# denix56/SI-Mamba

Hardware: AMD Instinct MI355X
Metric: point-clouds/sec (fwd+bwd) (higher is better)
Workload: dtype f32; 1 GPU; PointMamba classifier train step (FPS+kNN grouping, encoder, spectral SAST ordering, 12 Mamba blocks d=384 at L=1024, head, AdamW), 1024 pts -> 128 patches; global_batch=64, per_gpu_batch=64, npoints=1024, patches=128, mamba_seq_len=1024, parallelism=dp1, communicator_ranks=1, library_gemm=tuned solution table (si_mamba_amd/tuned/gemm_gfx950.csv)

## Files before the change

include/simamba.h:

```cpp
#ifndef SIMAMBA_H_
#define SIMAMBA_H_

#include <stddef.h>

#ifdef __cplusplus
extern "C" {
#endif

#define SIMAMBA_ABI_VERSION 9

#define SIMAMBA_F32  0
#define SIMAMBA_BF16 1

#define SIMAMBA_OK            0
#define SIMAMBA_E_NULLPTR    -1
#define SIMAMBA_E_SHAPE      -2
#define SIMAMBA_E_DTYPE      -3
#define SIMAMBA_E_DSTATE     -4
#define SIMAMBA_E_WIDTH      -5
#define SIMAMBA_E_WORKSPACE  -6
#define SIMAMBA_E_GROUPS     -7
#define SIMAMBA_E_ALIGN      -8
#define SIMAMBA_E_VARIANT    -9
#define SIMAMBA_E_BIAS       -10
// ... 74 lines not shown
                         void* stream);
int simamba_conv_xdt_proj_fwd(const void* x, const float* cw, const float* cb, const void* wx, const void* wdt,
                              void* xconv, void* xdbl, void* delta, int batch, int D, int seqlen, int S, int R,
                              int io_dtype, long long x_bstride, void* stream);

int simamba_seq_gather_fwd(const void* in, const int* idx, void* out, int batch, int channels, int G, int L,
                           long long out_bstride, int io_dtype, void* stream);
int simamba_seq_gather_bwd(const void* dout, const int* inv, void* din, int batch, int channels, int G, int L,
                           int R, long long dout_bstride, int io_dtype, void* stream);

int simamba_causal_conv1d_fwd(const void* x, const float* w, const float* bias, void* out,
                              int batch, int dim, int seqlen, int width, int silu,
                              int io_dtype, long long x_bstride, void* stream);
int simamba_causal_conv1d_bwd(const void* x, const float* w, const float* bias,
                              const void* dout, void* dx, float* dw, float* dbias,
                              int batch, int dim, int seqlen, int width, int silu,
                              int io_dtype, long long x_bstride, long long dx_bstride, void* stream);
long long simamba_causal_conv1d_bwd_workspace_floats(int batch, int dim, int seqlen, int width, int flags);
int simamba_causal_conv1d_bwd_ex(const void* x, const float* w, const float* bias,
                                 const void* dout, void* dx, float* dw, float* dbias,
                                 int batch, int dim, int seqlen, int width, int silu,
                                 int io_dtype, long long x_bstride, long long dx_bstride, int flags,
                                 float* workspace, long long workspace_floats, void* stream);

int simamba_add_layer_norm_grid(int batch, int rows_per_batch);
int simamba_add_layer_norm_fwd(const void* hidden, const float* residual, const float* rowscale,
                               const float* weight, const float* bias, float* residual_out,
                               void* normed, float* mean, float* rstd, int batch, int rows_per_batch,
                               int dim, float eps, int hidden_dtype, int out_dtype, void* stream);
int simamba_add_layer_norm_bwd(const void* dnormed, const float* dresidual_out,
                               const float* residual_out, const float* mean, const float* rstd,
                               const float* weight, const float* rowscale, float* dresidual,
                               void* dhidden, float* dwb_partial, int batch, int rows_per_batch,
                               int dim, int hidden_dtype, int out_dtype, void* stream);

#define SIMAMBA_NORM_RMS 1
int simamba_add_layer_norm_fwd_ex(const void* hidden, const float* residual, const float* rowscale,
                                  const float* weight, const float* bias, float* residual_out,
                                  void* normed, float* mean, float* rstd, int batch, int rows_per_batch,
                                  int dim, float eps, int hidden_dtype, int out_dtype, int flags, void* stream);
int simamba_add_layer_norm_bwd_ex(const void* dnormed, const float* dresidual_out,
                                  const float* residual_out, const float* mean, const float* rstd,
                                  const float* weight, const float* rowscale, float* dresidual,
                                  void* dhidden, float* dwb_partial, int batch, int rows_per_batch,
                                  int dim, int hidden_dtype, int out_dtype, int flags, void* stream);

// ... 203 lines not shown
```

si_mamba_amd/_lib.py:

```python
from __future__ import annotations

import ctypes
import os
from ctypes import c_char_p, c_float, c_int, c_longlong, c_size_t, c_uint, c_void_p

_HERE = os.path.dirname(os.path.abspath(__file__))
LIB_PATH = os.path.join(_HERE, "libsimamba_hip.so")

F32, BF16 = 0, 1

SPEC_SYMMETRIC = 0x01
SPEC_SELF_LOOP = 0x02
SPEC_BINARY = 0x04
SPEC_MATRIX_SYM = 0x08
SPEC_SMALLEST = 0x10
SPEC_SIGMA_MEAN = 0x20
SPEC_LARGE_G = 0x40
SPEC_MAX_G = 128
SPEC_MAX_G_LARGE = 512

SCAN_AUTO, SCAN_ROWSCAN, SCAN_LPC2, SCAN_LPC4, SCAN_MIX = 0, 1, 2, 4, 6
CKPT_ROW, CKPT_SEQ = 128, 16
BWD_DETERMINISTIC = 1
NORM_RMS = 1
# ... 34 lines not shown
                                              _LL, _LL, _LL, _LL, _LL, c_int, c_int, _P, _LL, _P]),
    "simamba_selective_scan_dt_fwd": (c_int, [_P, _P, _P, _P, _P, _P, _P, _P, _P, _P,
                                              c_int, c_int, c_int, c_int, c_int, c_int,
                                              _LL, _LL, _LL, c_int, c_int, _P]),
    "simamba_selective_scan_dt_bwd": (c_int, [_P, _P, _P, _P, _P, _P, _P, _P, _P,
                                              _P, _P, _P, _P, _P, _P, _P, _P,
                                              c_int, c_int, c_int, c_int, c_int, c_int,
                                              _LL, _LL, _LL, _LL, _P]),
    "simamba_selective_scan_dt_bwd_ex": (c_int, [_P, _P, _P, _P, _P, _P, _P, _P, _P,
                                                 _P, _P, _P, _P, _P, _P, _P, _P,
                                                 c_int, c_int, c_int, c_int, c_int, c_int,
                                                 _LL, _LL, _LL, _LL, c_int, _P, _LL, _P]),
    "simamba_xdt_proj_fwd": (c_int, [_P, _P, _P, _P, _P, c_int, c_int, c_int, c_int, c_int, c_int, _LL, _P]),
    "simamba_conv_xdt_proj_fwd": (c_int, [_P, _P, _P, _P, _P, _P, _P, _P, c_int, c_int, c_int, c_int, c_int, c_int, _LL,
                                          _P]),
    "simamba_seq_gather_fwd": (c_int, [_P, _P, _P, c_int, c_int, c_int, c_int, _LL, c_int, _P]),
    "simamba_seq_gather_bwd": (c_int, [_P, _P, _P, c_int, c_int, c_int, c_int, c_int, _LL, c_int, _P]),
    "simamba_causal_conv1d_fwd": (c_int, [_P, _P, _P, _P, c_int, c_int, c_int, c_int, c_int, c_int, _LL, _P]),
    "simamba_causal_conv1d_bwd": (c_int, [_P, _P, _P, _P, _P, _P, _P,
                                          c_int, c_int, c_int, c_int, c_int, c_int, _LL, _LL, _P]),
    "simamba_causal_conv1d_bwd_workspace_floats": (_LL, [c_int, c_int, c_int, c_int, c_int]),
    "simamba_causal_conv1d_bwd_ex": (c_int, [_P, _P, _P, _P, _P, _P, _P,
                                             c_int, c_int, c_int, c_int, c_int, c_int, _LL, _LL, c_int, _P, _LL, _P]),
    "simamba_add_layer_norm_grid": (c_int, [c_int, c_int]),
    "simamba_add_layer_norm_fwd": (c_int, [_P, _P, _P, _P, _P, _P, _P, _P, _P, c_int, c_int, c_int, c_float,
                                           c_int, c_int, _P]),
    "simamba_add_layer_norm_bwd": (c_int, [_P, _P, _P, _P, _P, _P, _P, _P, _P, _P, c_int, c_int, c_int,
                                           c_int, c_int, _P]),
    "simamba_add_layer_norm_fwd_ex": (c_int, [_P, _P, _P, _P, _P, _P, _P, _P, _P, c_int, c_int, c_int, c_float,
                                              c_int, c_int, c_int, _P]),
    "simamba_add_layer_norm_bwd_ex": (c_int, [_P, _P, _P, _P, _P, _P, _P, _P, _P, _P, c_int, c_int, c_int,
                                              c_int, c_int, c_int, _P]),
    "simamba_add_layer_norm_check_slots": (c_int, [_P, c_int, c_int]),
    "simamba_add_layer_norm_fwd_slots": (c_int, [_P, _P, _P, _P, _P, _P, _P, _P, _P, _P, c_int, _P, c_int, c_int, c_int,
                                                 c_int, c_float, c_int, c_int, c_int, _P]),
    "simamba_add_layer_norm_bwd_slots": (c_int, [_P, _P, _P, _P, _P, _P, _P, _P, _P, _P, _P, c_int, _P, c_int, c_int,
                                                 c_int, c_int, c_int, c_int, c_int, _P]),
    "simamba_out_proj_add_ln_fwd": (c_int, [_P, _P, _P, _P, _P, _P, _P, _P, _P, _P, c_int, c_int, c_int, c_int, c_float,
                                            c_int, _P]),
    "simamba_out_proj_add_ln_fwd_ex": (c_int, [_P, _P, _P, _P, _P, _P, _P, _P, _P, _P, c_int, c_int, c_int, c_int,
                                               c_float, c_int, c_int, _P]),
    "simamba_in_proj_fwd": (c_int, [_P, _P, _P, c_int, c_int, c_int, c_int, c_int, _P]),
    "simamba_bn_relu_grid": (c_int, [_LL]),
    "simamba_bn_relu_fwd": (c_int, [_P, _P, c_int, _P, _P, _P, _P, c_float, c_float, c_int, _P, _P, _P, _P, _LL, c_int,
                                    _LL, c_int, _P]),
    "simamba_bn_relu_bwd": (c_int, [_P, _P, _P, c_int, _P, _P, _P, _P, _P, _P, c_int, _P, _P, _P, _LL, c_int, _LL,
# ... 313 lines not shown
    step = scan_plan_step(batch, dim, seqlen, dstate, dtype, **operands)
    count("scan_ckpt_seq" if step == CKPT_SEQ else "scan_ckpt_row")
    if not need_grad:
        return step, None
    n = load().simamba_scan_ckpt_floats(batch, dim, seqlen, dstate, step)
    return step, (torch.empty(n, device=device, dtype=torch.float32) if n else None)


def scan_bwd_accumulators(batch, dim, seqlen, dstate, has_D, has_bias, device):
    import torch
    sizes = [dim * dstate, batch * dstate * seqlen, batch * dstate * seqlen, dim if has_D else 0,
             dim if has_bias else 0]
    flat = torch.empty(sum(sizes), device=device, dtype=torch.float32)
    parts, o = [], 0
    for n in sizes:
        parts.append(flat[o:o + n])
        o += n
    dA = parts[0].view(dim, dstate)
    dB = parts[1].view(batch, dstate, seqlen)
    dC = parts[2].view(batch, dstate, seqlen)
    return dA, dB, dC, (parts[3] if has_D else None), (parts[4] if has_bias else None)


_deterministic = [None]


def set_deterministic(on):
    _deterministic[0] = _tristate(on)


class deterministic(_Override):
    cell, coerce = _deterministic, staticmethod(_tristate)


def deterministic_enabled():
    if _deterministic[0] is not None:
        return _deterministic[0]
    import torch
    return torch.are_deterministic_algorithms_enabled()


def det_args(workspace_query, *dims, device):
    if not deterministic_enabled():
        return 0, None, 0
    import torch
    n_floats = workspace_query(*dims, BWD_DETERMINISTIC)
# ... 4 lines not shown
```

si_mamba_amd/csrc/add_norm.hip:

```cpp
#include "common.h"

namespace simamba {

constexpr int kLnThreads = 256;
constexpr int kLnMaxChunks = 8;

struct LnArgs {
  const void* hidden;
  const float* residual;
  const float* rowscale;
  const float* weight;
  const float* bias;
  float* residual_out;
  void* normed;
  float* mean;
  float* rstd;
  const void* dnormed;
  const float* dresidual_out;
  float* dresidual;
  void* dhidden;
  float* dwb_partial;
  const int* hidden_slot;
  const int* normed_slot;
  int hidden_batch, normed_batch;
  int batch, rows_per_batch, dim;
  float eps;
};

template <typename T>
__device__ __forceinline__ float4 ld4(const T* p) {
  const Pack<T, 4> pk = *reinterpret_cast<const Pack<T, 4>*>(p);
  return make_float4(to_f32<T>(pk.v[0]), to_f32<T>(pk.v[1]), to_f32<T>(pk.v[2]), to_f32<T>(pk.v[3]));
}
template <typename T>
__device__ __forceinline__ void st4(T* p, float4 v) {
  Pack<T, 4> pk;
  pk.v[0] = from_f32<T>(v.x); pk.v[1] = from_f32<T>(v.y); pk.v[2] = from_f32<T>(v.z); pk.v[3] = from_f32<T>(v.w);
  *reinterpret_cast<Pack<T, 4>*>(p) = pk;
}

__device__ __forceinline__ int ln_slot(const int* __restrict__ map, int b, int count) {
  if (!map) return b;
  const int s = __builtin_amdgcn_readfirstlane(map[b]);
  return (s >= 0 && s < count) ? s : -1;
}

struct LnRow {
  int b, hs, os;
};
__device__ __forceinline__ LnRow ln_row(const LnArgs& p, int row) {
  LnRow r;
  r.b = __builtin_amdgcn_readfirstlane(row / p.rows_per_batch);
  r.hs = ln_slot(p.hidden_slot, r.b, p.hidden_batch);
  r.os = ln_slot(p.normed_slot, r.b, p.normed_batch);
  return r;
}

template <typename TH, typename TO, int kChunks, bool kRms>
__global__ __launch_bounds__(kLnThreads) void add_ln_fwd_kernel(LnArgs p) {
  const bool slots = p.hidden_slot || p.normed_slot;
  const int lane = threadIdx.x & 63;
  const int wave_global = (blockIdx.x * kLnThreads + threadIdx.x) >> 6;
  const int nwaves = (gridDim.x * kLnThreads) >> 6;
  const int rows = p.batch * p.rows_per_batch;
  const int nch = p.dim >> 2;
  const TH* __restrict__ hg = static_cast<const TH*>(p.hidden);
  TO* __restrict__ og = static_cast<TO*>(p.normed);
  float4 w[kChunks], bs[kChunks];
#pragma unroll
  for (int k = 0; k < kChunks; ++k) {
    const int c = lane + 64 * k;
    w[k] = c < nch ? *reinterpret_cast<const float4*>(p.weight + 4 * c) : make_float4(0, 0, 0, 0);
    bs[k] = (!kRms && c < nch && p.bias) ? *reinterpret_cast<const float4*>(p.bias + 4 * c) : make_float4(0, 0, 0, 0);
  }
  const float inv_dim = 1.f / p.dim;
  LnRow next = (slots && wave_global < rows) ? ln_row(p, wave_global) : LnRow{0, 0, 0};
  for (int row = wave_global; row < rows; row += nwaves) {
    const size_t base = static_cast<size_t>(row) * p.dim;
    const float scale = (p.rowscale && p.residual) ? p.rowscale[row / p.rows_per_batch] : 1.f;
    size_t hbase = base, obase = base;
    bool has_h = true, has_o = true;
    if (slots) {
      const LnRow cur = next;
      const int ahead = row + nwaves;
      next = ln_row(p, ahead < rows ? ahead : row);
      const int r = __builtin_amdgcn_readfirstlane(row) - cur.b * p.rows_per_batch;
      has_h = cur.hs >= 0; has_o = cur.os >= 0;
      hbase = (static_cast<size_t>(has_h ? cur.hs : 0) * p.rows_per_batch + r) * p.dim;
      obase = (static_cast<size_t>(has_o ? cur.os : 0) * p.rows_per_batch + r) * p.dim;
    }
    float4 x[kChunks];
    float sum = 0.f;
#pragma unroll
    for (int k = 0; k < kChunks; ++k) {
      const int c = lane + 64 * k;
      if (c < nch) {
        float4 h;
        if (!has_h) {
          h = *reinterpret_cast<const float4*>(p.residual + base + 4 * c);
        } else {
          h = ld4<TH>(hg + hbase + 4 * c);
          if (p.residual) {
            const float4 r = *reinterpret_cast<const float4*>(p.residual + base + 4 * c);
            h.x = fmaf(h.x, scale, r.x); h.y = fmaf(h.y, scale, r.y);
            h.z = fmaf(h.z, scale, r.z); h.w = fmaf(h.w, scale, r.w);
          }
        }
        if (p.residual_out) *reinterpret_cast<float4*>(p.residual_out + base + 4 * c) = h;
        x[k] = h;
        sum += (h.x + h.y) + (h.z + h.w);
      } else {
        x[k] = make_float4(0, 0, 0, 0);
// ... 30 lines not shown
}

template <typename TH, typename TO, int kChunks, bool kRms>
__global__ __launch_bounds__(kLnThreads) void add_ln_bwd_kernel(LnArgs p) {
  const bool slots = p.hidden_slot || p.normed_slot;
  extern __shared__ float sred[];
  const int lane = threadIdx.x & 63;
  const int wave = threadIdx.x >> 6;
  const int wave_global = (blockIdx.x * kLnThreads + threadIdx.x) >> 6;
  const int nwaves = (gridDim.x * kLnThreads) >> 6;
  const int rows = p.batch * p.rows_per_batch;
  const int nch = p.dim >> 2;
  const TO* __restrict__ dyg = static_cast<const TO*>(p.dnormed);
  TH* __restrict__ dhg = static_cast<TH*>(p.dhidden);
  float4 w[kChunks], dw[kChunks], db[kChunks];
#pragma unroll
  for (int k = 0; k < kChunks; ++k) {
    const int c = lane + 64 * k;
    w[k] = c < nch ? *reinterpret_cast<const float4*>(p.weight + 4 * c) : make_float4(0, 0, 0, 0);
    dw[k] = make_float4(0, 0, 0, 0);
    db[k] = make_float4(0, 0, 0, 0);
  }
  const float inv_dim = 1.f / p.dim;
  LnRow next = (slots && wave_global < rows) ? ln_row(p, wave_global) : LnRow{0, 0, 0};
  for (int row = wave_global; row < rows; row += nwaves) {
    const size_t base = static_cast<size_t>(row) * p.dim;
    size_t hbase = base, obase = base;
    bool has_h = true, has_o = true;
    if (slots) {
      const LnRow cur = next;
      const int ahead = row + nwaves;
      next = ln_row(p, ahead < rows ? ahead : row);
      const int r = __builtin_amdgcn_readfirstlane(row) - cur.b * p.rows_per_batch;
      has_h = cur.hs >= 0; has_o = cur.os >= 0;
      hbase = (static_cast<size_t>(has_h ? cur.hs : 0) * p.rows_per_batch + r) * p.dim;
      obase = (static_cast<size_t>(has_o ? cur.os : 0) * p.rows_per_batch + r) * p.dim;
    }
    if (!has_o) {
      const float scale = (p.rowscale && dhg) ? p.rowscale[row / p.rows_per_batch] : 1.f;
#pragma unroll
      for (int k = 0; k < kChunks; ++k) {
        const int c = lane + 64 * k;
        if (c < nch) {
          const float4 dx = p.dresidual_out ? *reinterpret_cast<const float4*>(p.dresidual_out + base + 4 * c)
                                            : make_float4(0, 0, 0, 0);
          if (p.dresidual) *reinterpret_cast<float4*>(p.dresidual + base + 4 * c) = dx;
          if (dhg && has_h)
            st4<TH>(dhg + hbase + 4 * c, make_float4(dx.x * scale, dx.y * scale, dx.z * scale, dx.w * scale));
        }
      }
      continue;
    }
    const float mean = kRms ? 0.f : p.mean[row], rstd = p.rstd[row];
    float4 xh[kChunks], g[kChunks];
    float s1 = 0.f, s2 = 0.f;
#pragma unroll
    for (int k = 0; k < kChunks; ++k) {
      const int c = lane + 64 * k;
      if (c < nch) {
        const float4 x = *reinterpret_cast<const float4*>(p.residual_out + base + 4 * c);
        const float4 dy = ld4<TO>(dyg + obase + 4 * c);
        xh[k] = make_float4((x.x - mean) * rstd, (x.y - mean) * rstd, (x.z - mean) * rstd, (x.w - mean) * rstd);
        g[k] = make_float4(dy.x * w[k].x, dy.y * w[k].y, dy.z * w[k].z, dy.w * w[k].w);
        dw[k].x = fmaf(dy.x, xh[k].x, dw[k].x); dw[k].y = fmaf(dy.y, xh[k].y, dw[k].y);
        dw[k].z = fmaf(dy.z, xh[k].z, dw[k].z); dw[k].w = fmaf(dy.w, xh[k].w, dw[k].w);
        db[k].x += dy.x; db[k].y += dy.y; db[k].z += dy.z; db[k].w += dy.w;
        s1 += (g[k].x + g[k].y) + (g[k].z + g[k].w);
        s2 += (g[k].x * xh[k].x + g[k].y * xh[k].y) + (g[k].z * xh[k].z + g[k].w * xh[k].w);
      } else {
        xh[k] = make_float4(0, 0, 0, 0);
        g[k] = make_float4(0, 0, 0, 0);
      }
    }
    const float c1 = kRms ? 0.f : wave_allreduce_sum(s1) * inv_dim;
    const float c2 = wave_allreduce_sum(s2) * inv_dim;
    const float scale = (p.rowscale && dhg) ? p.rowscale[row / p.rows_per_batch] : 1.f;
#pragma unroll
    for (int k = 0; k < kChunks; ++k) {
      const int c = lane + 64 * k;
      if (c < nch) {
        float4 dx;
        dx.x = (g[k].x - c1 - xh[k].x * c2) * rstd;
        dx.y = (g[k].y - c1 - xh[k].y * c2) * rstd;
        dx.z = (g[k].z - c1 - xh[k].z * c2) * rstd;
        dx.w = (g[k].w - c1 - xh[k].w * c2) * rstd;
        if (p.dresidual_out) {
          const float4 r = *reinterpret_cast<const float4*>(p.dresidual_out + base + 4 * c);
          dx.x += r.x; dx.y += r.y; dx.z += r.z; dx.w += r.w;
        }
        if (p.dresidual) *reinterpret_cast<float4*>(p.dresidual + base + 4 * c) = dx;
        if (dhg && has_h)
          st4<TH>(dhg + hbase + 4 * c, make_float4(dx.x * scale, dx.y * scale, dx.z * scale, dx.w * scale));
      }
    }
  }
  float* mine = sred + wave * 2 * p.dim;
#pragma unroll
  for (int k = 0; k < kChunks; ++k) {
    const int c = lane + 64 * k;
    if (c < nch) {
      *reinterpret_cast<float4*>(mine + 4 * c) = dw[k];
      if (!kRms) *reinterpret_cast<float4*>(mine + p.dim + 4 * c) = db[k];
    }
  }
  __syncthreads();
  float* out = p.dwb_partial + static_cast<size_t>(blockIdx.x) * 2 * p.dim;
  for (int i = threadIdx.x; i < (kRms ? 1 : 2) * p.dim; i += kLnThreads) {
    float v = 0.f;
#pragma unroll
    for (int wv = 0; wv < kLnThreads / 64; ++wv) v += sred[wv * 2 * p.dim + i];
    out[i] = v;
  }
}

static int ln_grid(int rows) {
  int g = (rows + 3) / 4;
  return g < 1 ? 1 : (g > 1024 ? 1024 : g);
}

template <typename TH, typename TO, bool kRms>
static int launch_ln(const LnArgs& a, bool bwd, int grid, hipStream_t s) {
  const int chunks = ((a.dim >> 2) + 63) / 64;
#define SIMAMBA_LN_CASE(K)                                                                                      \
  if (chunks <= K) {                                                                                             \
    if (bwd)                                                                                                     \
      hipLaunchKernelGGL((add_ln_bwd_kernel<TH, TO, K, kRms>), dim3(grid), dim3(kLnThreads),                     \
                         sizeof(float) * (kLnThreads / 64) * 2 * a.dim, s, a);                                   \
    else                                                                                                         \
      hipLaunchKernelGGL((add_ln_fwd_kernel<TH, TO, K, kRms>), dim3(grid), dim3(kLnThreads), 0, s, a);           \
    return static_cast<int>(hipGetLastError());                                                                  \
  }
  SIMAMBA_LN_CASE(1)
  SIMAMBA_LN_CASE(2)
  SIMAMBA_LN_CASE(4)
  SIMAMBA_LN_CASE(8)
#undef SIMAMBA_LN_CASE
  return SIMAMBA_E_SHAPE;
}

template <typename TH, typename TO>
static int launch_ln(const LnArgs& a, bool bwd, bool rms, int grid, hipStream_t s) {
  return rms ? launch_ln<TH, TO, true>(a, bwd, grid, s) : launch_ln<TH, TO, false>(a, bwd, grid, s);
}

static int dispatch_ln(const LnArgs& a, bool bwd, bool rms, int grid, int hidden_dtype, int out_dtype, hipStream_t s) {
  if (hidden_dtype == SIMAMBA_F32 && out_dtype == SIMAMBA_F32) return launch_ln<float, float>(a, bwd, rms, grid, s);
  if (hidden_dtype == SIMAMBA_BF16 && out_dtype == SIMAMBA_BF16)
    return launch_ln<bf16_t, bf16_t>(a, bwd, rms, grid, s);
  if (hidden_dtype == SIMAMBA_F32 && out_dtype == SIMAMBA_BF16) return launch_ln<float, bf16_t>(a, bwd, rms, grid, s);
  if (hidden_dtype == SIMAMBA_BF16 && out_dtype == SIMAMBA_F32) return launch_ln<bf16_t, float>(a, bwd, rms, grid, s);
  return SIMAMBA_E_DTYPE;
}
// ... 126 lines not shown
```

si_mamba_amd/csrc/det_reduce.h:

```cpp
#pragma once
#include <hip/hip_runtime.h>

namespace simamba {

struct DetSumJob {
  const float* part;
  float* out;
  long long kstride;
  long long n;
  int K;
};

constexpr int kDetSumMaxJobs = 5;

int det_sum_launch(const DetSumJob* jobs, int njobs, hipStream_t s);

}
```

si_mamba_amd/csrc/det_reduce.hip:

```cpp
#include "det_reduce.h"

namespace simamba {

constexpr int kDetSumThreads = 256;
constexpr int kDetSumPerBlock = 4 * kDetSumThreads;

struct DetSumArgs {
  DetSumJob job[kDetSumMaxJobs];
  int vec[kDetSumMaxJobs];
  int blk0[kDetSumMaxJobs + 1];
  int njobs;
};

__global__ __launch_bounds__(kDetSumThreads) void det_sum_kernel(DetSumArgs a) {
  const int blk = blockIdx.x;
  int j = 0;
#pragma unroll
  for (int q = 1; q < kDetSumMaxJobs; ++q) j = (q < a.njobs && blk >= a.blk0[q]) ? q : j;
  const float* __restrict__ part = a.job[j].part;
  float* __restrict__ out = a.job[j].out;
  const long long ks = a.job[j].kstride, n = a.job[j].n;
  const int K = a.job[j].K;
  const long long i0 = (static_cast<long long>(blk - a.blk0[j]) * kDetSumThreads + threadIdx.x) * 4;
  if (i0 >= n) return;
  if (a.vec[j] && i0 + 4 <= n) {
    const float* p = part + i0;
    float4 acc = make_float4(0.f, 0.f, 0.f, 0.f);
    int k = 0;
    for (; k + 4 <= K; k += 4) {
      float4 v[4];
#pragma unroll
      for (int m = 0; m < 4; ++m) v[m] = *reinterpret_cast<const float4*>(p + (k + m) * ks);
#pragma unroll
      for (int m = 0; m < 4; ++m) {
        acc.x += v[m].x; acc.y += v[m].y; acc.z += v[m].z; acc.w += v[m].w;
      }
    }
    for (; k < K; ++k) {
      const float4 v = *reinterpret_cast<const float4*>(p + k * ks);
      acc.x += v.x; acc.y += v.y; acc.z += v.z; acc.w += v.w;
    }
    *reinterpret_cast<float4*>(out + i0) = acc;
    return;
  }
  for (long long i = i0; i < n && i < i0 + 4; ++i) {
    float acc = 0.f;
    for (int k = 0; k < K; ++k) acc += part[k * ks + i];
    out[i] = acc;
  }
}

int det_sum_launch(const DetSumJob* jobs, int njobs, hipStream_t s) {
  DetSumArgs a{};
  int blocks = 0, m = 0;
  for (int i = 0; i < njobs && m < kDetSumMaxJobs; ++i) {
    if (jobs[i].n <= 0) continue;
    a.job[m] = jobs[i];
    a.vec[m] = (reinterpret_cast<uintptr_t>(jobs[i].part) & 15u) == 0 && (reinterpret_cast<uintptr_t>(jobs[i].out) & 15u) == 0 &&
               jobs[i].kstride % 4 == 0;
    a.blk0[m] = blocks;
    blocks += static_cast<int>((jobs[i].n + kDetSumPerBlock - 1) / kDetSumPerBlock);
    ++m;
  }
  if (!m) return static_cast<int>(hipSuccess);
  a.njobs = m;
  for (int q = m; q <= kDetSumMaxJobs; ++q) a.blk0[q] = blocks;
  hipLaunchKernelGGL(det_sum_kernel, dim3(blocks), dim3(kDetSumThreads), 0, s, a);
  return static_cast<int>(hipGetLastError());
}

}
```

si_mamba_amd/mamba_inner.py:

```python
from __future__ import annotations

import torch

from . import _lib


def _w(t, dtype):
    return t if t.dtype == dtype else t.to(dtype)


def _wx(W, X):
    return torch.bmm(W.unsqueeze(0).expand(X.shape[0], -1, -1), X)


def _xw(X, W):
    return torch.bmm(X, W.unsqueeze(0).expand(X.shape[0], -1, -1))


def _sum_bmm(X, Y):
    return torch.bmm(X, Y).sum(0, dtype=torch.float32)


class InProjFn(torch.autograd.Function):

    @staticmethod
    def forward(ctx, hidden, weight, bias):
        io = hidden.dtype
        if torch.is_autocast_enabled("cuda"):
            io = torch.get_autocast_dtype("cuda")
            hidden = hidden.to(io)
        wc = _w(weight, io)
        xz = tokens_times_weight(hidden, wc) if bias is None else _wx(wc, hidden.transpose(1, 2))
        if bias is not None:
            xz = xz + _w(bias, io)[None, :, None]
        ctx.save_for_backward(hidden, weight)
        ctx.wc = wc
        ctx.has_bias = bias is not None
        return xz

    @staticmethod
    def backward(ctx, dxz):
        hidden, weight = ctx.saved_tensors
        io = hidden.dtype
        dxz = dxz.to(io)
        dh = _xw(dxz.transpose(1, 2), ctx.wc) if ctx.needs_input_grad[0] else None
        dw = _sum_bmm(dxz, hidden).to(weight.dtype) if ctx.needs_input_grad[1] else None
        db = dxz.sum((0, 2)).to(weight.dtype) if ctx.has_bias else None
        return dh, dw, db


def tokens_times_weight(x, w):
    if (x.dtype in (torch.bfloat16, torch.float32) and w.dtype == x.dtype and x.is_cuda and x.dim() == 3
            and x.is_contiguous() and in_proj_hand_ok(x, w)):
        Bsz, L, C = x.shape
        wcc = w.contiguous()
        out = torch.empty(Bsz, w.shape[0], L, device=x.device, dtype=x.dtype)
        _lib.call("simamba_in_proj_fwd", x, wcc, out, Bsz, L, C, w.shape[0], _lib.dtype_code(x.dtype),
                  device=x.device, time_as="in_proj_fwd")
        _lib.count("in_proj_hand")
        return out
    return _wx(w, x.transpose(1, 2))


def in_proj_hand_ok(hidden, wc):
    Bsz, L, C = hidden.shape
    tile = 128 if hidden.dtype == torch.float32 else 256
    return (C % 64 == 0 and C <= 384 and wc.shape[0] % 32 == 0 and L % 8 == 0 and hidden.data_ptr() % 16 == 0
            and _lib.in_proj_hand_enabled(Bsz * ((L + tile - 1) // tile), hidden.dtype))

# ... 109 lines not shown
                            dt_proj_w.dtype, None if no_out else out_proj_w.dtype, A.dtype,
                            None if D is None else D.dtype, None if delta_bias is None else delta_bias.dtype)
        ctx.save_for_backward(xz, x_conv, x_dbl, delta, None if no_out else y, cw, cb, x_proj_w, dt_proj_w, out_proj_w,
                              Af, Df, bf, x_ckpt)
        return out

    @staticmethod
    def backward(ctx, dout):
        (xz, x_conv, x_dbl, delta, y, cw, cb, x_proj_w, dt_proj_w, out_proj_w, Af, Df, bf, x_ckpt) = ctx.saved_tensors
        lib = _lib.load()
        R, N, W = ctx.dims
        io = xz.dtype
        code = _lib.dtype_code(io)
        Bsz, twoD, L = xz.shape
        Dm = twoD // 2
        S = R + 2 * N
        dev = xz.device
        xbs = xz.stride(0)
        dout = dout.to(io)
        f32 = dict(device=dev, dtype=torch.float32)
        xw_c, dtw_c, ow_c = ctx.wcast
        if ctx.no_out:
            dy = dout.contiguous()
            d_out_w = d_out_b = None
        else:
            if dout.stride(2) != 1:
                dout = dout.contiguous()
            d_out_w = _sum_bmm(dout.transpose(1, 2), y.transpose(1, 2))
            d_out_b = dout.sum((0, 1)) if ctx.has_out_bias else None
            dy = tokens_times_weight(dout, ow_c.t())

        dxz = torch.empty_like(xz)
        du = torch.empty(Bsz, Dm, L, device=dev, dtype=io)
        ddelta = torch.empty(Bsz, Dm, L, device=dev, dtype=io)
        dA, dB, dC, dD, dbias = _lib.scan_bwd_accumulators(Bsz, Dm, L, N, Df is not None, bf is not None, dev)
        Bv, Cv = x_dbl[:, :, R:R + N], x_dbl[:, :, R + N:]
        z, dz = xz[:, Dm:], dxz[:, Dm:]
        flags, ws, nws = _lib.det_args(lib.simamba_scan_bwd_workspace_floats, Bsz, Dm, L, N,
                                       _lib.CKPT_SEQ if ctx.dtw_k is not None else ctx.ckpt_step, device=dev)
        _lib.count("scan_bwd_det" if flags else "scan_bwd_atomic")
        if ctx.dtw_k is not None:
            _lib.call("simamba_selective_scan_dt_bwd_ex", x_conv, x_dbl, ctx.dtw_k, Af, Df, z, bf, dy, x_ckpt,
                      du, ddelta, dA, dB, dC, dD, dz, dbias, Bsz, Dm, L, N, R, code,
                      xbs, dxz.stride(0), x_dbl.stride(0), x_dbl.stride(1), flags, ws, nws,
                      device=dev, time_as="scan_bwd")
        else:
            _lib.call("simamba_selective_scan_bwd_ex", x_conv, delta, Af, Bv, Cv, Df, z, bf, dy, x_ckpt,
                      du, ddelta, dA, dB, dC, dD, dz, dbias, Bsz, Dm, L, N, code, 1,
                      xbs, dxz.stride(0), x_dbl.stride(0), 1, x_dbl.stride(1), ctx.ckpt_step, flags, ws, nws,
                      device=dev, time_as="scan_bwd")

        dx_dbl = torch.empty(Bsz, L, S, device=dev, dtype=io)
        dx_dbl[:, :, :R].copy_(_xw(ddelta.transpose(1, 2), dtw_c))
        dBC = torch.as_strided(dB, (2, Bsz, N, L), (Bsz * N * L, N * L, L, 1))
        dx_dbl[:, :, R:].view(Bsz, L, 2, N).copy_(dBC.permute(1, 3, 0, 2))
        d_dt_w = _sum_bmm(ddelta, x_dbl[:, :, :R])
        d_x_w = _sum_bmm(dx_dbl.transpose(1, 2), x_conv.transpose(1, 2))
        wxT = xw_c.t().unsqueeze(0).expand(Bsz, -1, -1)
        torch.baddbmm(du, wxT, dx_dbl.transpose(1, 2), out=du)

        dconv = torch.empty(Dm * W + (Dm if cb is not None else 0), **f32)
        dcw = dconv[:Dm * W].view(Dm, W)
        dcb = dconv[Dm * W:] if cb is not None else None
        flags, ws, nws = _lib.det_args(lib.simamba_causal_conv1d_bwd_workspace_floats, Bsz, Dm, L, W, device=dev)
        _lib.count("conv1d_bwd_det" if flags else "conv1d_bwd_atomic")
        _lib.call("simamba_causal_conv1d_bwd_ex", xz, cw, cb, du, dxz, dcw, dcb, Bsz, Dm, L, W, 1, code,
                  xbs, dxz.stride(0), flags, ws, nws, device=dev, time_as="conv1d_bwd")

        t_cw, t_cb, t_xw, t_dtw, t_ow, t_A, t_D, t_b = ctx.param_dtypes
        return (dxz, dcw.to(t_cw), None if dcb is None else dcb.to(t_cb), d_x_w.to(t_xw), d_dt_w.to(t_dtw),
                None if d_out_w is None else d_out_w.to(t_ow),
                None if d_out_b is None else d_out_b.to(out_proj_w.dtype), dA.to(t_A),
                None if dD is None else dD.to(t_D), None if dbias is None else dbias.to(t_b), None, None, None)


def mamba_inner_fn(xz, conv1d_weight, conv1d_bias, x_proj_weight, delta_proj_weight, out_proj_weight,
                   out_proj_bias, A, D=None, delta_bias=None, dt_rank=None, d_state=None):
    if conv1d_weight.dim() == 3:
        conv1d_weight = conv1d_weight.squeeze(1)
    if dt_rank is None:
# ... 6 lines not shown
```

si_mamba_amd/out_norm.py:

```python
from __future__ import annotations

import torch

from . import _lib
from .add_norm import add_norm_bwd
from .mamba_inner import _sum_bmm, tokens_times_weight


def out_proj_add_ln_ok(y, out_w, d_model):
    B, D, L = y.shape
    return (y.is_cuda and y.dtype == torch.bfloat16 and y.stride(2) == 1 and y.stride(1) == L and y.stride(0) == D * L
            and d_model % 128 == 0 and d_model <= 384 and D % 64 == 0 and L % 8 == 0 and D * L * 2 < 2 ** 32 - 65536
            and tuple(out_w.shape) == (d_model, D) and y.data_ptr() % 16 == 0)


class OutProjAddLnFn(torch.autograd.Function):
    @staticmethod
    def forward(ctx, y, out_w, residual, ln_w, ln_b, eps, rowscale, out_dtype, rms=False):
        _lib.require_gpu(y, "out_proj_add_ln_fn")
        Bsz, D, L = y.shape
        C = out_w.shape[0]
        dev = y.device
        flags = _lib.NORM_RMS if rms else 0
        wc = out_w.to(torch.bfloat16).contiguous()
# ... 4 lines not shown
        res_out = torch.empty(Bsz, L, C, device=dev, dtype=torch.float32)
        normed = torch.empty(Bsz, L, C, device=dev, dtype=out_dtype)
        mean = None if rms else torch.empty(Bsz * L, device=dev, dtype=torch.float32)
        rstd = torch.empty(Bsz * L, device=dev, dtype=torch.float32)
        _lib.call("simamba_out_proj_add_ln_fwd_ex", y, wc, res, rs, lw, lb, res_out, normed, mean, rstd, Bsz, D, L, C,
                  float(eps), _lib.dtype_code(out_dtype), flags, device=dev,
                  time_as="out_proj_add_rms_fwd" if rms else "out_proj_add_ln_fwd")
        ctx.save_for_backward(y, wc, res_out, mean, rstd, lw, rs)
        ctx.meta = (Bsz, L, C, _lib.dtype_code(out_dtype), residual is not None,
                    None if residual is None else residual.dtype, ln_w.dtype, ln_b is not None, out_w.dtype, flags)
        return normed, res_out

    @staticmethod
    def backward(ctx, dnormed, dres_out):
        y, wc, res_out, mean, rstd, lw, rs = ctx.saved_tensors
        Bsz, L, C, ocode, has_res, res_dtype, lwdtype, has_bias, owdtype, flags = ctx.meta
        dev = y.device
        dn = dnormed.contiguous()
        dro = None if dres_out is None else dres_out.float().contiguous()
        dres = torch.empty(res_out.shape, device=dev, dtype=torch.float32) if has_res else None
        dhid = torch.empty(res_out.shape, device=dev, dtype=torch.bfloat16)
        dwb = add_norm_bwd(dn, dro, res_out, mean, rstd, lw, rs, dres, dhid, Bsz, L, C, _lib.BF16, ocode, flags)
        dy = tokens_times_weight(dhid, wc.t())
        d_out_w = _sum_bmm(dhid.transpose(1, 2), y.transpose(1, 2))
        return (dy, d_out_w.to(owdtype), None if not has_res else dres.to(res_dtype), dwb[0].to(lwdtype),
                dwb[1].to(lwdtype) if has_bias else None, None, None, None, None)


def out_proj_add_ln_fn(y, out_w, residual, ln_w, ln_b, eps=1e-5, rowscale=None, out_dtype=torch.bfloat16, rms=False):
    if rms and ln_b is not None:
        raise ValueError("out_proj_add_ln_fn(rms=True): RMSNorm takes no bias")
    return OutProjAddLnFn.apply(y, out_w, residual, ln_w, ln_b, eps, rowscale, out_dtype, bool(rms))
```

Measured before the change: 1169 point-clouds/s.

## Batch weight-gradient partial sums into one multi-job kernel and table LN row lookups

Replaces the per-weight torch `.sum(0)` over batched bmm partials with a custom multi-job reduction kernel that handles several weight-gradient reductions (fp32 or bf16 partials) in one launch, with more loads in flight per thread. It also precomputes the LayerNorm slot and rowscale lookups into an LDS table and walks rows incrementally instead of dividing per row. The aim is fewer kernel launches and less reduction overhead in the backward pass. The risks are lower occupancy from the smaller 64-thread blocks, extra LDS use, and deferring the out-proj weight sum so its bmm output stays alive longer.

```diff
diff --git a/include/simamba.h b/include/simamba.h
--- a/include/simamba.h
+++ b/include/simamba.h
@@ -120,6 +120,10 @@
                                  int batch, int dim, int seqlen, int width, int silu,
                                  int io_dtype, long long x_bstride, long long dx_bstride, int flags,
                                  float* workspace, long long workspace_floats, void* stream);
+
+#define SIMAMBA_BATCH_SUM_MAX_JOBS 8
+int simamba_batch_sum(const void* const* part, float* const* out, const long long* kstride, const long long* n,
+                      const int* K, const int* part_dtype, int njobs, void* stream);
 
 int simamba_add_layer_norm_grid(int batch, int rows_per_batch);
 int simamba_add_layer_norm_fwd(const void* hidden, const float* residual, const float* rowscale,
diff --git a/si_mamba_amd/_lib.py b/si_mamba_amd/_lib.py
--- a/si_mamba_amd/_lib.py
+++ b/si_mamba_amd/_lib.py
@@ -80,6 +80,7 @@
     "simamba_causal_conv1d_bwd_workspace_floats": (_LL, [c_int, c_int, c_int, c_int, c_int]),
     "simamba_causal_conv1d_bwd_ex": (c_int, [_P, _P, _P, _P, _P, _P, _P,
                                              c_int, c_int, c_int, c_int, c_int, c_int, _LL, _LL, c_int, _P, _LL, _P]),
+    "simamba_batch_sum": (c_int, [_P, _P, _P, _P, _P, _P, c_int, _P]),
     "simamba_add_layer_norm_grid": (c_int, [c_int, c_int]),
     "simamba_add_layer_norm_fwd": (c_int, [_P, _P, _P, _P, _P, _P, _P, _P, _P, c_int, c_int, c_int, c_float,
                                            c_int, c_int, _P]),
@@ -439,6 +440,44 @@
     return dA, dB, dC, (parts[3] if has_D else None), (parts[4] if has_bias else None)
 
 
+BATCH_SUM_MAX_JOBS = 8
+_batch_sum = [True]
+sum_counters = {}
+
+
+class batch_sum_route(_Override):
+    cell = _batch_sum
+
+
+def _batch_sum_takes(p):
+    import torch
+    return (_batch_sum[0] and p.is_cuda and p.dtype in (torch.float32, torch.bfloat16) and p.dim() >= 1
+            and p.shape[0] > 0 and p[0].is_contiguous())
+
+
+def sum_partials(parts):
+    import torch
+    outs, jobs = [None] * len(parts), {}
+    for i, p in enumerate(parts):
+        if _batch_sum_takes(p):
+            outs[i] = torch.empty(p.shape[1:], device=p.device, dtype=torch.float32)
+            jobs.setdefault(p.device, []).append((p, outs[i]))
+        else:
+            sum_counters["batch_sum_aten"] = sum_counters.get("batch_sum_aten", 0) + 1
+            outs[i] = p.sum(0, dtype=torch.float32)
+    for dev, todo in jobs.items():
+        for s in range(0, len(todo), BATCH_SUM_MAX_JOBS):
+            chunk = todo[s:s + BATCH_SUM_MAX_JOBS]
+            n = len(chunk)
+            call("simamba_batch_sum",
+                 (c_void_p * n)(*[p.data_ptr() for p, _ in chunk]), (c_void_p * n)(*[o.data_ptr() for _, o in chunk]),
+                 (c_longlong * n)(*[p.stride(0) for p, _ in chunk]), (c_longlong * n)(*[o.numel() for _, o in chunk]),
+                 (c_int * n)(*[p.shape[0] for p, _ in chunk]), (c_int * n)(*[dtype_code(p.dtype) for p, _ in chunk]),
+                 n, device=dev, time_as="batch_sum")
+            sum_counters["batch_sum"] = sum_counters.get("batch_sum", 0) + 1
+    return outs
+
+
 _deterministic = [None]
 
 
diff --git a/si_mamba_amd/csrc/add_norm.hip b/si_mamba_amd/csrc/add_norm.hip
--- a/si_mamba_amd/csrc/add_norm.hip
+++ b/si_mamba_amd/csrc/add_norm.hip
@@ -41,19 +41,67 @@
 
 __device__ __forceinline__ int ln_slot(const int* __restrict__ map, int b, int count) {
   if (!map) return b;
-  const int s = __builtin_amdgcn_readfirstlane(map[b]);
+  const int s = map[b];
   return (s >= 0 && s < count) ? s : -1;
 }
 
+constexpr int kLnTable = 1024;
+struct LnTable {
+  int *hs, *os;
+  float* scale;
+};
+__device__ __forceinline__ LnTable ln_table_at(void* lds, int batch) {
+  LnTable t;
+  t.hs = static_cast<int*>(lds);
+  t.os = t.hs + batch;
+  t.scale = reinterpret_cast<float*>(t.os + batch);
+  return t;
+}
+__device__ __forceinline__ void ln_table_fill(const LnArgs& p, const LnTable& t) {
+  for (int b = threadIdx.x; b < p.batch; b += kLnThreads) {
+    t.hs[b] = ln_slot(p.hidden_slot, b, p.hidden_batch);
+    t.os[b] = ln_slot(p.normed_slot, b, p.normed_batch);
+    t.scale[b] = p.rowscale ? p.rowscale[b] : 1.f;
+  }
+  __syncthreads();
+}
+
 struct LnRow {
-  int b, hs, os;
+  int b, r, hs, os;
+  float scale;
 };
-__device__ __forceinline__ LnRow ln_row(const LnArgs& p, int row) {
-  LnRow r;
-  r.b = __builtin_amdgcn_readfirstlane(row / p.rows_per_batch);
-  r.hs = ln_slot(p.hidden_slot, r.b, p.hidden_batch);
-  r.os = ln_slot(p.normed_slot, r.b, p.normed_batch);
-  return r;
+__device__ __forceinline__ LnRow ln_row(const LnArgs& p, const LnTable& t, bool table, int b, int r) {
+  LnRow x;
+  x.b = b; x.r = r;
+  int hs, os;
+  float scale;
+  if (table) {
+    hs = t.hs[b]; os = t.os[b]; scale = t.scale[b];
+  } else {
+    hs = ln_slot(p.hidden_slot, b, p.hidden_batch);
+    os = ln_slot(p.normed_slot, b, p.normed_batch);
+    scale = p.rowscale ? p.rowscale[b] : 1.f;
+  }
+  x.hs = __builtin_amdgcn_readfirstlane(hs);
+  x.os = __builtin_amdgcn_readfirstlane(os);
+  x.scale = __builtin_bit_cast(float, __builtin_amdgcn_readfirstlane(__builtin_bit_cast(int, scale)));
+  return x;
+}
+
+struct LnWalk {
+  int b, r, db, dr;
+};
+__device__ __forceinline__ LnWalk ln_walk_begin(int row, int nwaves, int rows_per_batch) {
+  LnWalk w;
+  w.b = __builtin_amdgcn_readfirstlane(row / rows_per_batch);
+  w.r = __builtin_amdgcn_readfirstlane(row - w.b * rows_per_batch);
+  w.db = nwaves / rows_per_batch;
+  w.dr = nwaves - w.db * rows_per_batch;
+  return w;
+}
+__device__ __forceinline__ void ln_walk_step(LnWalk& w, int rows_per_batch) {
+  w.b += w.db; w.r += w.dr;
+  if (w.r >= rows_per_batch) { w.r -= rows_per_batch; ++w.b; }
 }
 
 template <typename TH, typename TO, int kChunks, bool kRms>
@@ -74,20 +122,30 @@
     bs[k] = (!kRms && c < nch && p.bias) ? *reinterpret_cast<const float4*>(p.bias + 4 * c) : make_float4(0, 0, 0, 0);
   }
   const float inv_dim = 1.f / p.dim;
-  LnRow next = (slots && wave_global < rows) ? ln_row(p, wave_global) : LnRow{0, 0, 0};
+  const bool lookups = slots || p.rowscale;
+  const bool table = lookups && p.batch <= kLnTable;
+  extern __shared__ float sred[];
+  const LnTable tab = ln_table_at(sred, p.batch);
+  if (table) ln_table_fill(p, tab);
+  LnWalk walk = ln_walk_begin(wave_global < rows ? wave_global : 0, nwaves, p.rows_per_batch);
+  LnRow next = (lookups && wave_global < rows) ? ln_row(p, tab, table, walk.b, walk.r) : LnRow{0, 0, 0, 0, 1.f};
   for (int row = wave_global; row < rows; row += nwaves) {
     const size_t base = static_cast<size_t>(row) * p.dim;
-    const float scale = (p.rowscale && p.residual) ? p.rowscale[row / p.rows_per_batch] : 1.f;
+    float scale = 1.f;
     size_t hbase = base, obase = base;
     bool has_h = true, has_o = true;
-    if (slots) {
+    if (lookups) {
       const LnRow cur = next;
-      const int ahead = row + nwaves;
-      next = ln_row(p, ahead < rows ? ahead : row);
-      const int r = __builtin_amdgcn_readfirstlane(row) - cur.b * p.rows_per_batch;
-      has_h = cur.hs >= 0; has_o = cur.os >= 0;
-      hbase = (static_cast<size_t>(has_h ? cur.hs : 0) * p.rows_per_batch + r) * p.dim;
-      obase = (static_cast<size_t>(has_o ? cur.os : 0) * p.rows_per_batch + r) * p.dim;
+      if (row + nwaves < rows) {
+        ln_walk_step(walk, p.rows_per_batch);
+        next = ln_row(p, tab, table, walk.b, walk.r);
+      }
+      if (p.residual) scale = cur.scale;
+      if (slots) {
+        has_h = cur.hs >= 0; has_o = cur.os >= 0;
+        hbase = (static_cast<size_t>(has_h ? cur.hs : 0) * p.rows_per_batch + cur.r) * p.dim;
+        obase = (static_cast<size_t>(has_o ? cur.os : 0) * p.rows_per_batch + cur.r) * p.dim;
+      }
     }
     float4 x[kChunks];
     float sum = 0.f;
@@ -164,22 +222,31 @@
     db[k] = make_float4(0, 0, 0, 0);
   }
   const float inv_dim = 1.f / p.dim;
-  LnRow next = (slots && wave_global < rows) ? ln_row(p, wave_global) : LnRow{0, 0, 0};
+  const bool lookups = slots || p.rowscale;
+  const bool table = lookups && p.batch <= kLnTable;
+  const LnTable tab = ln_table_at(sred + (kLnThreads / 64) * 2 * p.dim, p.batch);
+  if (table) ln_table_fill(p, tab);
+  LnWalk walk = ln_walk_begin(wave_global < rows ? wave_global : 0, nwaves, p.rows_per_batch);
+  LnRow next = (lookups && wave_global < rows) ? ln_row(p, tab, table, walk.b, walk.r) : LnRow{0, 0, 0, 0, 1.f};
   for (int row = wave_global; row < rows; row += nwaves) {
     const size_t base = static_cast<size_t>(row) * p.dim;
+    float scale = 1.f;
     size_t hbase = base, obase = base;
     bool has_h = true, has_o = true;
-    if (slots) {
+    if (lookups) {
       const LnRow cur = next;
-      const int ahead = row + nwaves;
-      next = ln_row(p, ahead < rows ? ahead : row);
-      const int r = __builtin_amdgcn_readfirstlane(row) - cur.b * p.rows_per_batch;
-      has_h = cur.hs >= 0; has_o = cur.os >= 0;
-      hbase = (static_cast<size_t>(has_h ? cur.hs : 0) * p.rows_per_batch + r) * p.dim;
-      obase = (static_cast<size_t>(has_o ? cur.os : 0) * p.rows_per_batch + r) * p.dim;
+      if (row + nwaves < rows) {
+        ln_walk_step(walk, p.rows_per_batch);
+        next = ln_row(p, tab, table, walk.b, walk.r);
+      }
+      if (dhg) scale = cur.scale;
+      if (slots) {
+        has_h = cur.hs >= 0; has_o = cur.os >= 0;
+        hbase = (static_cast<size_t>(has_h ? cur.hs : 0) * p.rows_per_batch + cur.r) * p.dim;
+        obase = (static_cast<size_t>(has_o ? cur.os : 0) * p.rows_per_batch + cur.r) * p.dim;
+      }
     }
     if (!has_o) {
-      const float scale = (p.rowscale && dhg) ? p.rowscale[row / p.rows_per_batch] : 1.f;
 #pragma unroll
       for (int k = 0; k < kChunks; ++k) {
         const int c = lane + 64 * k;
@@ -216,7 +283,6 @@
     }
     const float c1 = kRms ? 0.f : wave_allreduce_sum(s1) * inv_dim;
     const float c2 = wave_allreduce_sum(s2) * inv_dim;
-    const float scale = (p.rowscale && dhg) ? p.rowscale[row / p.rows_per_batch] : 1.f;
 #pragma unroll
     for (int k = 0; k < kChunks; ++k) {
       const int c = lane + 64 * k;
@@ -255,6 +321,11 @@
   }
 }
 
+static size_t ln_table_bytes(const LnArgs& a) {
+  const bool lookups = a.hidden_slot || a.normed_slot || a.rowscale;
+  return (lookups && a.batch <= kLnTable) ? 3 * sizeof(int) * static_cast<size_t>(a.batch) : 0;
+}
+
 static int ln_grid(int rows) {
   int g = (rows + 3) / 4;
   return g < 1 ? 1 : (g > 1024 ? 1024 : g);
@@ -267,9 +338,10 @@
   if (chunks <= K) {                                                                                             \
     if (bwd)                                                                                                     \
       hipLaunchKernelGGL((add_ln_bwd_kernel<TH, TO, K, kRms>), dim3(grid), dim3(kLnThreads),                     \
-                         sizeof(float) * (kLnThreads / 64) * 2 * a.dim, s, a);                                   \
+                         sizeof(float) * (kLnThreads / 64) * 2 * a.dim + ln_table_bytes(a), s, a);               \
     else                                                                                                         \
-      hipLaunchKernelGGL((add_ln_fwd_kernel<TH, TO, K, kRms>), dim3(grid), dim3(kLnThreads), 0, s, a);           \
+      hipLaunchKernelGGL((add_ln_fwd_kernel<TH, TO, K, kRms>), dim3(grid), dim3(kLnThreads), ln_table_bytes(a),  \
+                         s, a);                                                                                  \
     return static_cast<int>(hipGetLastError());                                                                  \
   }
   SIMAMBA_LN_CASE(1)
diff --git a/si_mamba_amd/csrc/det_reduce.h b/si_mamba_amd/csrc/det_reduce.h
--- a/si_mamba_amd/csrc/det_reduce.h
+++ b/si_mamba_amd/csrc/det_reduce.h
@@ -1,17 +1,20 @@
 #pragma once
 #include <hip/hip_runtime.h>
+
+#include "../../include/simamba.h"
 
 namespace simamba {
 
 struct DetSumJob {
-  const float* part;
+  const void* part;
   float* out;
   long long kstride;
   long long n;
   int K;
+  int bf16;
 };
 
-constexpr int kDetSumMaxJobs = 5;
+constexpr int kDetSumMaxJobs = SIMAMBA_BATCH_SUM_MAX_JOBS;
 
 int det_sum_launch(const DetSumJob* jobs, int njobs, hipStream_t s);
 
diff --git a/si_mamba_amd/csrc/det_reduce.hip b/si_mamba_amd/csrc/det_reduce.hip
--- a/si_mamba_amd/csrc/det_reduce.hip
+++ b/si_mamba_amd/csrc/det_reduce.hip
@@ -1,9 +1,11 @@
+#include "common.h"
 #include "det_reduce.h"
 
 namespace simamba {
 
-constexpr int kDetSumThreads = 256;
+constexpr int kDetSumThreads = 64;
 constexpr int kDetSumPerBlock = 4 * kDetSumThreads;
+constexpr int kDetSumInFlight = 16;
 
 struct DetSumArgs {
   DetSumJob job[kDetSumMaxJobs];
@@ -12,43 +14,60 @@
   int njobs;
 };
 
+template <typename T>
+__device__ __forceinline__ float4 det_ld4(const T* p) {
+  const Pack<T, 4> pk = *reinterpret_cast<const Pack<T, 4>*>(p);
+  return make_float4(to_f32<T>(pk.v[0]), to_f32<T>(pk.v[1]), to_f32<T>(pk.v[2]), to_f32<T>(pk.v[3]));
+}
+
+template <typename T, int kN>
+__device__ __forceinline__ void det_sum_step(const T* p, long long ks, int k, float4& acc) {
+  float4 v[kN];
+#pragma unroll
+  for (int m = 0; m < kN; ++m) v[m] = det_ld4<T>(p + (k + m) * ks);
+#pragma unroll
+  for (int m = 0; m < kN; ++m) {
+    acc.x += v[m].x; acc.y += v[m].y; acc.z += v[m].z; acc.w += v[m].w;
+  }
+}
+
+template <typename T>
+__device__ __forceinline__ void det_sum_outputs(const DetSumJob& job, int vec, long long i0) {
+  const T* __restrict__ part = static_cast<const T*>(job.part);
+  float* __restrict__ out = job.out;
+  const long long ks = job.kstride, n = job.n;
+  const int K = job.K;
+  if (vec && i0 + 4 <= n) {
+    const T* p = part + i0;
+    float4 acc = make_float4(0.f, 0.f, 0.f, 0.f);
+    int k = 0;
+    for (; k + kDetSumInFlight <= K; k += kDetSumInFlight) det_sum_step<T, kDetSumInFlight>(p, ks, k, acc);
+    for (; k + 4 <= K; k += 4) det_sum_step<T, 4>(p, ks, k, acc);
+    for (; k < K; ++k) det_sum_step<T, 1>(p, ks, k, acc);
+    *reinterpret_cast<float4*>(out + i0) = acc;
+    return;
+  }
+  for (long long i = i0; i < n && i < i0 + 4; ++i) {
+    float acc = 0.f;
+    for (int k = 0; k < K; ++k) acc += to_f32<T>(part[k * ks + i]);
+    out[i] = acc;
+  }
+}
+
 __global__ __launch_bounds__(kDetSumThreads) void det_sum_kernel(DetSumArgs a) {
   const int blk = blockIdx.x;
   int j = 0;
 #pragma unroll
   for (int q = 1; q < kDetSumMaxJobs; ++q) j = (q < a.njobs && blk >= a.blk0[q]) ? q : j;
-  const float* __restrict__ part = a.job[j].part;
-  float* __restrict__ out = a.job[j].out;
-  const long long ks = a.job[j].kstride, n = a.job[j].n;
-  const int K = a.job[j].K;
   const long long i0 = (static_cast<long long>(blk - a.blk0[j]) * kDetSumThreads + threadIdx.x) * 4;
-  if (i0 >= n) return;
-  if (a.vec[j] && i0 + 4 <= n) {
-    const float* p = part + i0;
-    float4 acc = make_float4(0.f, 0.f, 0.f, 0.f);
-    int k = 0;
-    for (; k + 4 <= K; k += 4) {
-      float4 v[4];
-#pragma unroll
-      for (int m = 0; m < 4; ++m) v[m] = *reinterpret_cast<const float4*>(p + (k + m) * ks);
-#pragma unroll
-      for (int m = 0; m < 4; ++m) {
-        acc.x += v[m].x; acc.y += v[m].y; acc.z += v[m].z; acc.w += v[m].w;
-      }
-    }
-    for (; k < K; ++k) {
-      const float4 v = *reinterpret_cast<const float4*>(p + k * ks);
-      acc.x += v.x; acc.y += v.y; acc.z += v.z; acc.w += v.w;
-    }
-    *reinterpret_cast<float4*>(out + i0) = acc;
-    return;
-  }
-  for (long long i = i0; i < n && i < i0 + 4; ++i) {
-    float acc = 0.f;
-    for (int k = 0; k < K; ++k) acc += part[k * ks + i];
-    out[i] = acc;
-  }
+  if (i0 >= a.job[j].n) return;
+  if (a.job[j].bf16)
+    det_sum_outputs<bf16_t>(a.job[j], a.vec[j], i0);
+  else
+    det_sum_outputs<float>(a.job[j], a.vec[j], i0);
 }
+
+static long long det_sum_blocks(long long n) { return (n + kDetSumPerBlock - 1) / kDetSumPerBlock; }
 
 int det_sum_launch(const DetSumJob* jobs, int njobs, hipStream_t s) {
   DetSumArgs a{};
@@ -56,10 +75,11 @@
   for (int i = 0; i < njobs && m < kDetSumMaxJobs; ++i) {
     if (jobs[i].n <= 0) continue;
     a.job[m] = jobs[i];
-    a.vec[m] = (reinterpret_cast<uintptr_t>(jobs[i].part) & 15u) == 0 && (reinterpret_cast<uintptr_t>(jobs[i].out) & 15u) == 0 &&
-               jobs[i].kstride % 4 == 0;
+    const uintptr_t pmask = jobs[i].bf16 ? 7u : 15u;
+    a.vec[m] = (reinterpret_cast<uintptr_t>(jobs[i].part) & pmask) == 0 &&
+               (reinterpret_cast<uintptr_t>(jobs[i].out) & 15u) == 0 && jobs[i].kstride % 4 == 0;
     a.blk0[m] = blocks;
-    blocks += static_cast<int>((jobs[i].n + kDetSumPerBlock - 1) / kDetSumPerBlock);
+    blocks += static_cast<int>(det_sum_blocks(jobs[i].n));
     ++m;
   }
   if (!m) return static_cast<int>(hipSuccess);
@@ -70,3 +90,23 @@
 }
 
 }
+
+using namespace simamba;
+
+extern "C" int simamba_batch_sum(const void* const* part, float* const* out, const long long* kstride,
+                                 const long long* n, const int* K, const int* part_dtype, int njobs, void* stream) {
+  if (njobs < 0 || njobs > SIMAMBA_BATCH_SUM_MAX_JOBS) return SIMAMBA_E_SHAPE;
+  if (njobs == 0) return SIMAMBA_OK;
+  if (!part || !out || !kstride || !n || !K || !part_dtype) return SIMAMBA_E_NULLPTR;
+  DetSumJob jobs[SIMAMBA_BATCH_SUM_MAX_JOBS];
+  long long blocks = 0;
+  for (int i = 0; i < njobs; ++i) {
+    if (n[i] < 0 || K[i] < 0 || kstride[i] < 0 || (K[i] > 1 && kstride[i] < n[i])) return SIMAMBA_E_SHAPE;
+    if (part_dtype[i] != SIMAMBA_F32 && part_dtype[i] != SIMAMBA_BF16) return SIMAMBA_E_DTYPE;
+    if (n[i] > 0 && (!out[i] || (K[i] > 0 && !part[i]))) return SIMAMBA_E_NULLPTR;
+    blocks += det_sum_blocks(n[i]);
+    if (blocks > 0x7fffffffll) return SIMAMBA_E_SHAPE;
+    jobs[i] = DetSumJob{part[i], out[i], kstride[i], n[i], K[i], part_dtype[i] == SIMAMBA_BF16};
+  }
+  return det_sum_launch(jobs, njobs, static_cast<hipStream_t>(stream));
+}
diff --git a/si_mamba_amd/mamba_inner.py b/si_mamba_amd/mamba_inner.py
--- a/si_mamba_amd/mamba_inner.py
+++ b/si_mamba_amd/mamba_inner.py
@@ -17,8 +17,13 @@
     return torch.bmm(X, W.unsqueeze(0).expand(X.shape[0], -1, -1))
 
 
-def _sum_bmm(X, Y):
-    return torch.bmm(X, Y).sum(0, dtype=torch.float32)
+def _sum_bmm(*pairs):
+    todo = [i for i, xy in enumerate(pairs) if xy is not None]
+    sums = _lib.sum_partials([pairs[i] if torch.is_tensor(pairs[i]) else torch.bmm(*pairs[i]) for i in todo])
+    out = [None] * len(pairs)
+    for i, v in zip(todo, sums):
+        out[i] = v
+    return out
 
 
 class InProjFn(torch.autograd.Function):
@@ -44,7 +49,7 @@
         io = hidden.dtype
         dxz = dxz.to(io)
         dh = _xw(dxz.transpose(1, 2), ctx.wc) if ctx.needs_input_grad[0] else None
-        dw = _sum_bmm(dxz, hidden).to(weight.dtype) if ctx.needs_input_grad[1] else None
+        dw = _sum_bmm((dxz, hidden))[0].to(weight.dtype) if ctx.needs_input_grad[1] else None
         db = dxz.sum((0, 2)).to(weight.dtype) if ctx.has_bias else None
         return dh, dw, db
 
@@ -200,11 +205,11 @@
         xw_c, dtw_c, ow_c = ctx.wcast
         if ctx.no_out:
             dy = dout.contiguous()
-            d_out_w = d_out_b = None
+            out_w_pair = d_out_b = None
         else:
             if dout.stride(2) != 1:
                 dout = dout.contiguous()
-            d_out_w = _sum_bmm(dout.transpose(1, 2), y.transpose(1, 2))
+            out_w_pair = torch.bmm(dout.transpose(1, 2), y.transpose(1, 2))
             d_out_b = dout.sum((0, 1)) if ctx.has_out_bias else None
             dy = tokens_times_weight(dout, ow_c.t())
 
@@ -232,8 +237,8 @@
         dx_dbl[:, :, :R].copy_(_xw(ddelta.transpose(1, 2), dtw_c))
         dBC = torch.as_strided(dB, (2, Bsz, N, L), (Bsz * N * L, N * L, L, 1))
         dx_dbl[:, :, R:].view(Bsz, L, 2, N).copy_(dBC.permute(1, 3, 0, 2))
-        d_dt_w = _sum_bmm(ddelta, x_dbl[:, :, :R])
-        d_x_w = _sum_bmm(dx_dbl.transpose(1, 2), x_conv.transpose(1, 2))
+        d_out_w, d_dt_w, d_x_w = _sum_bmm(out_w_pair, (ddelta, x_dbl[:, :, :R]),
+                                          (dx_dbl.transpose(1, 2), x_conv.transpose(1, 2)))
         wxT = xw_c.t().unsqueeze(0).expand(Bsz, -1, -1)
         torch.baddbmm(du, wxT, dx_dbl.transpose(1, 2), out=du)
 
diff --git a/si_mamba_amd/out_norm.py b/si_mamba_amd/out_norm.py
--- a/si_mamba_amd/out_norm.py
+++ b/si_mamba_amd/out_norm.py
@@ -50,7 +50,7 @@
         dhid = torch.empty(res_out.shape, device=dev, dtype=torch.bfloat16)
         dwb = add_norm_bwd(dn, dro, res_out, mean, rstd, lw, rs, dres, dhid, Bsz, L, C, _lib.BF16, ocode, flags)
         dy = tokens_times_weight(dhid, wc.t())
-        d_out_w = _sum_bmm(dhid.transpose(1, 2), y.transpose(1, 2))
+        d_out_w, = _sum_bmm((dhid.transpose(1, 2), y.transpose(1, 2)))
         return (dy, d_out_w.to(owdtype), None if not has_res else dres.to(res_dtype), dwb[0].to(lwdtype),
                 dwb[1].to(lwdtype) if has_bias else None, None, None, None, None)
 
```

New measurement: 1177 point-clouds/s, median of 6. Within noise of the previous version (+0.6%).
